# casys-kaist/CoVA

Hardware: AMD Instinct MI355X
Metric: compressed-domain frames/sec (BlobNet+bboxcc) at 1080p b=256 (higher is better)
Workload: dtype f16

## Files before the change

cova_amd/csrc/bboxcc_wave.h:

```cpp
#pragma once
#include <cstdint>

#include "bboxcc_body.h"

#ifdef PHASE_TIMING
__device__ unsigned long long g_ccph[8];
#define CCWG_MARK(i)                                                        \
    do {                                                                    \
        if (tid == 0) {                                                     \
            const unsigned long long now_ = __builtin_amdgcn_s_memrealtime(); \
            atomicAdd(&g_ccph[i], now_ - cc_last_);                         \
            cc_last_ = now_;                                                \
        }                                                                   \
    } while (0)
#else
#define CCWG_MARK(i) do { } while (0)
#endif

namespace ccwave {

struct WvGeom {
    int H, W, BH, BW, NXB;
    int cap;
    int rows_bytes;
// ... 40 lines not shown
__device__ __forceinline__ uint64_t mask_upto(int e) { return e >= 63 ? ~0ull : ((2ull << e) - 1); }

__device__ __forceinline__ int frame_wave(const uint8_t *m, uint8_t *sm, const WvGeom &g, int area_thresh, covahip_box *ob,
                                           int32_t *count_out, int max_boxes, int lane) {
    uint32_t *rows = reinterpret_cast<uint32_t *>(sm);
    uint32_t *lab = reinterpret_cast<uint32_t *>(sm + g.rows_bytes);
    uint32_t *s_area = lab + g.cap, *s_minx = s_area + g.cap, *s_maxx = s_minx + g.cap, *s_miny = s_maxx + g.cap,
             *s_maxy = s_miny + g.cap;

    for (int i = lane; i < g.rows_bytes / 4; i += 64) rows[i] = 0;
    wave_fence();
    const int npieces = g.H * g.NXB;
    constexpr int UN = 8;
    for (int q0 = lane; q0 < npieces; q0 += 64 * UN) {
        uint2 v[UN];
#pragma unroll
        for (int k = 0; k < UN; k++) {
            const int q = q0 + 64 * k;
            v[k] = q < npieces ? *reinterpret_cast<const uint2 *>(m + (size_t)q * 8) : make_uint2(0, 0);
        }
#pragma unroll
        for (int k = 0; k < UN; k++) {
            if ((v[k].x | v[k].y) == 0) continue;
            const int q = q0 + 64 * k;
            const int y = g.mNXB ? (int)__umulhi((uint32_t)q, g.mNXB) : q, xc = q - y * g.NXB;
            const uint32_t tl = nz_bits(v[k].x), th = nz_bits(v[k].y);
            const uint32_t e = (((tl & 0x00800080u) * 0x00800100u) >> 30) | ((((th & 0x00800080u) * 0x00800100u) >> 30) << 2);
            const uint32_t o = (((tl & 0x80008000u) * 0x00008001u) >> 30) | ((((th & 0x80008000u) * 0x00008001u) >> 30) << 2);
            uint32_t *rw = rows + (y + 1) * 4 + (xc >> 3);
            const int sh = 4 * (xc & 7);
            if (e) atomicOr(rw, e << sh);
            if (o) atomicOr(rw + 2, o << sh);
        }
    }

    wave_fence();
    uint64_t a = 0, b = 0, c = 0, d = 0, ue = 0, uo = 0;
    if (lane < g.BH) {
        const uint4 ru = reinterpret_cast<const uint4 *>(rows)[2 * lane];
        const uint4 r0 = reinterpret_cast<const uint4 *>(rows)[2 * lane + 1];
        const uint4 r1 = reinterpret_cast<const uint4 *>(rows)[2 * lane + 2];
        ue = ru.x | ((uint64_t)ru.y << 32); uo = ru.z | ((uint64_t)ru.w << 32);
        a = r0.x | ((uint64_t)r0.y << 32);  b = r0.z | ((uint64_t)r0.w << 32);
        c = r1.x | ((uint64_t)r1.y << 32);  d = r1.z | ((uint64_t)r1.w << 32);
    }
    const uint64_t F = a | b | c | d;
    const uint64_t J = (a | c) & ((b | d) << 1);
    const uint64_t S = F & ~J;
    const int nr = __popcll((unsigned long long)S);
    int incl = nr;
#pragma unroll
    for (int o = 1; o < 64; o <<= 1) {
        const int t = __shfl_up(incl, o, 64);
        if (lane >= o) incl += t;
    }
    const int base = incl - nr;
    const int n = __shfl(incl, 63, 64);
    if (n > g.cap) return n;
    uint64_t S_up = (uint64_t)__shfl_up((unsigned long long)S, 1, 64), J_up = (uint64_t)__shfl_up((unsigned long long)J, 1, 64);
    int base_up = __shfl_up(base, 1, 64);
    if (lane == 0) { S_up = 0; J_up = 0; base_up = 0; }

    for (int i = lane; i < n; i += 64) lab[i] = (uint32_t)i;
    wave_fence();

    {
        const int nhelp = min(64 - g.BH, g.BH);
        const bool helper = lane >= g.BH && lane - g.BH < nhelp;
        const int row = helper ? lane - g.BH : lane;
        const bool split = row < nhelp;
        const uint64_t ha = (uint64_t)__shfl((unsigned long long)a, row, 64), hb = (uint64_t)__shfl((unsigned long long)b, row, 64);
        const uint64_t hc = (uint64_t)__shfl((unsigned long long)c, row, 64), hd = (uint64_t)__shfl((unsigned long long)d, row, 64);
        const uint64_t hue = (uint64_t)__shfl((unsigned long long)ue, row, 64), huo = (uint64_t)__shfl((unsigned long long)uo, row, 64);
        const uint64_t hSu = (uint64_t)__shfl((unsigned long long)S_up, row, 64), hJu = (uint64_t)__shfl((unsigned long long)J_up, row, 64);
        const int hbase = __shfl(base, row, 64), hbase_up = __shfl(base_up, row, 64);
        const uint64_t hJ = (ha | hc) & ((hb | hd) << 1);
        const uint64_t hS = (ha | hb | hc | hd) & ~hJ;
        const uint64_t hcU = (ha | hb) & (hue | huo), hcUL = ha & (huo << 1), hcUR = hb & (hue >> 1);
        uint64_t P = hS;
        P ^= P << 1; P ^= P << 2; P ^= P << 4; P ^= P << 8; P ^= P << 16; P ^= P << 32;
        uint64_t Sr = lane >= g.BH && !helper ? 0 : !split ? hS : helper ? hS & ~P : hS & P;
        while (__any(Sr != 0)) {
            uint64_t Tu = 0;
            int idx = 0;
            if (Sr) {
                const int s = ctz64(Sr);
                Sr &= Sr - 1;
                idx = hbase + __popcll((unsigned long long)(hS & ((1ull << s) - 1)));
                const uint64_t jr = (hJ >> s) >> 1;
                const int e = s + (~jr ? ctz64(~jr) : 0);
                const uint64_t mk = mask_upto(e) & ~((1ull << s) - 1);
                const uint64_t ra = ha & mk, rb = hb & mk, rc = hc & mk, rd = hd & mk;
                s_area[idx] = (uint32_t)(__popcll((unsigned long long)ra) + __popcll((unsigned long long)rb) +
                                         __popcll((unsigned long long)rc) + __popcll((unsigned long long)rd));
                s_minx[idx] = (uint32_t)(2 * s + (((ha | hc) >> s) & 1 ? 0 : 1));
                s_maxx[idx] = (uint32_t)(2 * e + (((hb | hd) >> e) & 1 ? 1 : 0));
                s_miny[idx] = (uint32_t)(2 * row + ((ra | rb) ? 0 : 1));
                s_maxy[idx] = (uint32_t)(2 * row + ((rc | rd) ? 1 : 0));
                Tu = (hcU & mk) | ((hcUL & mk) >> 1) | ((hcUR & mk) << 1);
            }
            while (__any(Tu != 0)) {
                if (Tu) {
                    const int p = ctz64(Tu);
                    const int rank = __popcll((unsigned long long)(hSu << (63 - p))) - 1;
                    const uint64_t jr = (hJu >> p) >> 1;
                    const int e_up = p + (~jr ? ctz64(~jr) : 0);
                    Tu &= ~mask_upto(e_up);
                    ccbody::uf_union(lab, (uint32_t)idx, (uint32_t)(hbase_up + rank));
                }
            }
        }
    }

    wave_fence();
    for (int i = lane; i < n; i += 64) {
        const uint32_t root = ccbody::uf_find(lab, (uint32_t)i);
        if (root != (uint32_t)i) {
            lab[i] = root;
            atomicAdd(&s_area[root], s_area[i]);
            atomicMin(&s_minx[root], s_minx[i]);
            atomicMax(&s_maxx[root], s_maxx[i]);
            atomicMin(&s_miny[root], s_miny[i]);
            atomicMax(&s_maxy[root], s_maxy[i]);
        }
    }
    wave_fence();
    int total = 0;
    for (int i0 = 0; i0 < n; i0 += 64) {
        const int i = i0 + lane;
        const bool keep = i < n && lab[i] == (uint32_t)i && (int)s_area[i] >= area_thresh;
        const uint64_t bal = __ballot(keep);
        if (keep) {
            const int pos = total + __popcll((unsigned long long)(bal & ((1ull << lane) - 1)));
            if (pos < max_boxes) {
                covahip_box bx;
                bx.left = (int32_t)s_minx[i];
                bx.top = (int32_t)s_miny[i];
                bx.width = (int32_t)(s_maxx[i] - s_minx[i] + 1);
                bx.height = (int32_t)(s_maxy[i] - s_miny[i] + 1);
                bx.area_px = (int32_t)s_area[i];
                ob[pos] = bx;
            }
        }
        total += __popcll((unsigned long long)bal);
    }
    if (lane == 0) *count_out = total;
    return n;
}

template <int NTH, bool PLANES = false>
__device__ __forceinline__ void frame_wg(const uint8_t *m, uint8_t *sm, const WvGeom &g, int area_thresh, covahip_box *ob,
                                         int32_t *count_out, int max_boxes, int tid, uint32_t *planes = nullptr) {
    constexpr int NWV = NTH / 64;
    const int lane = tid & 63, wave = tid >> 6;
    uint32_t *rows = PLANES ? planes : reinterpret_cast<uint32_t *>(sm);
    uint32_t *lab = reinterpret_cast<uint32_t *>(sm + g.rows_bytes);
    uint32_t *s_area = lab + g.cap, *s_minx = s_area + g.cap, *s_maxx = s_minx + g.cap, *s_miny = s_maxx + g.cap,
             *s_maxy = s_miny + g.cap;
    __shared__ uint32_t wave_tot[NWV];
#ifdef PHASE_TIMING
    unsigned long long cc_last_ = __builtin_amdgcn_s_memrealtime();
#endif

    if constexpr (!PLANES) {
    for (int i = tid; i < g.rows_bytes / 4; i += NTH) rows[i] = 0;
    __syncthreads();
    const int npieces = g.H * g.NXB;
    for (int q = tid; q < npieces; q += NTH) {
        const uint2 v = *reinterpret_cast<const uint2 *>(__builtin_assume_aligned(m + (size_t)q * 8, 8));
        if ((v.x | v.y) == 0) continue;
        const int y = g.mNXB ? (int)__umulhi((uint32_t)q, g.mNXB) : q, xc = q - y * g.NXB;
        const uint32_t tl = nz_bits(v.x), th = nz_bits(v.y);
        const uint32_t e = (((tl & 0x00800080u) * 0x00800100u) >> 30) | ((((th & 0x00800080u) * 0x00800100u) >> 30) << 2);
        const uint32_t o = (((tl & 0x80008000u) * 0x00008001u) >> 30) | ((((th & 0x80008000u) * 0x00008001u) >> 30) << 2);
        uint32_t *rw = rows + (y + 1) * 4 + (xc >> 3);
        const int sh = 4 * (xc & 7);
        if (e) atomicOr(rw, e << sh);
        if (o) atomicOr(rw + 2, o << sh);
    }
    __syncthreads();
    }
    CCWG_MARK(0);
    uint64_t a = 0, b = 0, c = 0, d = 0, ue = 0, uo = 0;
    if (lane < g.BH) {
        const uint4 ru = reinterpret_cast<const uint4 *>(rows)[2 * lane];
        const uint4 r0 = reinterpret_cast<const uint4 *>(rows)[2 * lane + 1];
        const uint4 r1 = reinterpret_cast<const uint4 *>(rows)[2 * lane + 2];
        ue = ru.x | ((uint64_t)ru.y << 32); uo = ru.z | ((uint64_t)ru.w << 32);
        a = r0.x | ((uint64_t)r0.y << 32);  b = r0.z | ((uint64_t)r0.w << 32);
        c = r1.x | ((uint64_t)r1.y << 32);  d = r1.z | ((uint64_t)r1.w << 32);
    }
    const uint64_t F = a | b | c | d;
    const uint64_t J = (a | c) & ((b | d) << 1);
    const uint64_t S = F & ~J;
    const uint64_t cU = (a | b) & (ue | uo), cUL = a & (uo << 1), cUR = b & (ue >> 1);
    const int nr = __popcll((unsigned long long)S);
    int incl = nr;
#pragma unroll
    for (int o = 1; o < 64; o <<= 1) {
        const int t = __shfl_up(incl, o, 64);
        if (lane >= o) incl += t;
    }
    const int base = incl - nr;
    const int n = __shfl(incl, 63, 64);
    uint64_t S_up = (uint64_t)__shfl_up((unsigned long long)S, 1, 64), J_up = (uint64_t)__shfl_up((unsigned long long)J, 1, 64);
    int base_up = __shfl_up(base, 1, 64);
    if (lane == 0) { S_up = 0; J_up = 0; base_up = 0; }
    for (int i = tid; i < n; i += NTH) lab[i] = (uint32_t)i;
    __syncthreads();
    CCWG_MARK(1);
    for (int k = wave; __any(k < nr); k += NWV) {
        uint64_t Tu = 0;
        const int idx = base + k;
        if (k < nr) {
            const int s = nth_set_bit64(S, k);
            const uint64_t jr = (J >> s) >> 1;
            const int e = s + (~jr ? ctz64(~jr) : 0);
            const uint64_t mk = mask_upto(e) & ~((1ull << s) - 1);
            const uint64_t ra = a & mk, rb = b & mk, rc = c & mk, rd = d & mk;
            s_area[idx] = (uint32_t)(__popcll((unsigned long long)ra) + __popcll((unsigned long long)rb) +
                                     __popcll((unsigned long long)rc) + __popcll((unsigned long long)rd));
            s_minx[idx] = (uint32_t)(2 * s + (((a | c) >> s) & 1 ? 0 : 1));
            s_maxx[idx] = (uint32_t)(2 * e + (((b | d) >> e) & 1 ? 1 : 0));
            s_miny[idx] = (uint32_t)(2 * lane + ((ra | rb) ? 0 : 1));
            s_maxy[idx] = (uint32_t)(2 * lane + ((rc | rd) ? 1 : 0));
            Tu = (cU & mk) | ((cUL & mk) >> 1) | ((cUR & mk) << 1);
        }
        while (__any(Tu != 0)) {
            if (Tu) {
                const int p = ctz64(Tu);
                const int rank = __popcll((unsigned long long)(S_up << (63 - p))) - 1;
                const uint64_t jr = (J_up >> p) >> 1;
                const int e_up = p + (~jr ? ctz64(~jr) : 0);
                Tu &= ~mask_upto(e_up);
                ccbody::uf_union(lab, (uint32_t)idx, (uint32_t)(base_up + rank));
            }
        }
    }
    __syncthreads();
    CCWG_MARK(2);
    for (int i = tid; i < n; i += NTH) {
        const uint32_t root = ccbody::uf_find(lab, (uint32_t)i);
        if (root != (uint32_t)i) {
            lab[i] = root;
            atomicAdd(&s_area[root], s_area[i]);
            atomicMin(&s_minx[root], s_minx[i]);
            atomicMax(&s_maxx[root], s_maxx[i]);
            atomicMin(&s_miny[root], s_miny[i]);
            atomicMax(&s_maxy[root], s_maxy[i]);
        }
    }
    __syncthreads();
    CCWG_MARK(3);
    const int per = (n + NTH - 1) / NTH;
    const int i0 = tid * per;
    uint32_t cnt = 0;
    for (int k = 0; k < per; k++) {
        const int i = i0 + k;
        if (i < n && lab[i] == (uint32_t)i && (int)s_area[i] >= area_thresh) cnt++;
    }
    uint32_t inc2 = cnt;
#pragma unroll
    for (int o = 1; o < 64; o <<= 1) {
        const uint32_t t = __shfl_up(inc2, o, 64);
        if (lane >= o) inc2 += t;
    }
    if (lane == 63) wave_tot[wave] = inc2;
    __syncthreads();
    uint32_t pbase = 0, total = 0;
#pragma unroll
    for (int k = 0; k < NWV; k++) {
        const uint32_t t = wave_tot[k];
        if (k < wave) pbase += t;
        total += t;
    }
    uint32_t pos = pbase + inc2 - cnt;
    for (int k = 0; k < per; k++) {
        const int i = i0 + k;
        if (i < n && lab[i] == (uint32_t)i && (int)s_area[i] >= area_thresh) {
            if ((int)pos < max_boxes) {
                covahip_box bx;
                bx.left = (int32_t)s_minx[i];
                bx.top = (int32_t)s_miny[i];
                bx.width = (int32_t)(s_maxx[i] - s_minx[i] + 1);
                bx.height = (int32_t)(s_maxy[i] - s_miny[i] + 1);
                bx.area_px = (int32_t)s_area[i];
                ob[pos] = bx;
            }
            pos++;
        }
    }
    if (tid == 0) *count_out = (int32_t)total;
    __syncthreads();
    CCWG_MARK(4);
}

}
```

cova_amd/csrc/blobnet_mfma.hip:

```cpp
#include <algorithm>
#include <cmath>
#include <cstdlib>
#include <cstring>
#include <mutex>
#include <type_traits>
#include <utility>
#include <vector>

#include "bboxcc_body.h"
#include "bboxcc_wave.h"
#include "blobnet.h"
#include "covahip_dev.h"

typedef _Float16 half8 __attribute__((ext_vector_type(8)));
typedef _Float16 half4 __attribute__((ext_vector_type(4)));
typedef float f32x16 __attribute__((ext_vector_type(16)));
typedef float f32x4 __attribute__((ext_vector_type(4)));
typedef _Float16 half2v __attribute__((ext_vector_type(2)));

namespace {

constexpr float BN_EPS = 1e-3f;
constexpr int WG = 256;

// ... 1603 lines not shown
    for (int i = tid; i < n_rows + n_cols; i += 512) {
        int piece;
        if (i < n_rows) {
            piece = i < RC ? i : (g.Hi + 1) * RC + (i - RC);
        } else {
            const int j = i - n_rows, y = j / (2 * CPP), k = j % (2 * CPP);
            piece = (y + 1) * RC + (k < CPP ? k : (g.Wi + 1) * CPP + (k - CPP));
        }
        *reinterpret_cast<uint4 *>(tile + piece * 16) = uint4{0, 0, 0, 0};
    }
}
template <int C1, int C2>
__device__ __forceinline__ void dec012_stage(uint8_t *tile, const __half *ss, const DecLvl &g, int wave, int lane, int first) {
    constexpr int C = C1 + C2, CPP = C / 8;
    const int RC = (g.Wi + 2) * CPP, NI = g.Wi * CPP;
    for (int y = (wave + 8 - first) & 7; y < g.Hi; y += 8) {
        const int r = y + 1;
        const __half *rowp = ss + (size_t)y * g.Wi * C2;
        uint8_t *rowl = tile + (r * RC + CPP) * 16;
        for (int q0 = 0; q0 < NI; q0 += 64) {
            const int q = q0 + lane;
            const int px = q / CPP, chp = q % CPP;
            const int cb = (chp ^ swz_eval<CPP>(g.swz, px + 1, r)) * 8;
            if (q < NI && cb >= C1) glds16(rowp + px * C2 + (cb - C1), rowl + q0 * 16);
        }
    }
}

template <int C, int COUT>
struct Dec012W {
    half8 wf[4 * (C / 16)];
    float es[16], eb[16];
};
template <int C, int COUT>
__device__ __forceinline__ void dec012_load(Dec012W<C, COUT> &w, const half8 *wfrag, const float *epi, int wave, int lane) {
    constexpr int MT = 4 * COUT / 32, KSTEPS = 4 * (C / 16);
    const int mtile = wave % MT, kh = lane >> 5;
    asm volatile("" : "+s"(wfrag), "+s"(epi));
#pragma unroll
    for (int ks = 0; ks < KSTEPS; ks++) w.wf[ks] = wfrag[(mtile * KSTEPS + ks) * 64 + lane];
#pragma unroll
    for (int gq = 0; gq < 4; gq++) {
        const int c0 = (mtile * 32 + 8 * gq + 4 * kh) % COUT;
        const float4 sc = *reinterpret_cast<const float4 *>(epi + c0), sh = *reinterpret_cast<const float4 *>(epi + COUT + c0);
        w.es[4 * gq] = sc.x; w.es[4 * gq + 1] = sc.y; w.es[4 * gq + 2] = sc.z; w.es[4 * gq + 3] = sc.w;
        w.eb[4 * gq] = sh.x; w.eb[4 * gq + 1] = sh.y; w.eb[4 * gq + 2] = sh.z; w.eb[4 * gq + 3] = sh.w;
    }
}
template <int C1, int C2, int COUT, int CN>
__device__ __forceinline__ void dec012_block(const uint8_t *lds0, const uint8_t *tile, uint8_t *next_tile, __half *gout, uint8_t *scr_base,
                                             const Dec012W<C1 + C2, COUT> &w, const DecLvl &g, const DecLvl &gn,
                                             int wave, int lane) {
    constexpr int C = C1 + C2, MT = 4 * COUT / 32, PG = 8 / MT;
    constexpr int KC = C / 16, KSTEPS = 4 * KC, CPP = C / 8, PS = C * 2;
    constexpr int AD = C == 128 ? 4 : 8;
    const int mtile = wave % MT, pgroup = wave / MT;
    const int TC = g.Wi + 2, GW = g.Wi + 1, GH = g.Hi + 1;
    const int kh = lane >> 5;
    const half8 (&wf)[KSTEPS] = w.wf;
    const float (&es)[16] = w.es, (&eb)[16] = w.eb;
    const int npos = GH * GW;
    const int ntiles = (npos + 31) / 32;
    for (int tile_i = pgroup; tile_i < ntiles; tile_i += PG) {
        const int q = tile_i * 32 + (lane & 31);
        const int qc = min(q, npos - 1);
        const int u = fdiv(qc, g.mGW), v = qc - u * GW;
        const uint32_t toff = (uint32_t)(uintptr_t)(lds_void *)tile;
        uint32_t pk[4];
#pragma unroll
        for (int tp = 0; tp < 4; tp++) {
            const int yy = u + 1 - (tp >> 1), xx = v + 1 - (tp & 1);
            pk[tp] = (toff + (uint32_t)((yy * TC + xx) * PS)) | (uint32_t)((kh ^ swz_eval<CPP>(g.swz, xx, yy)) << 4);
        }
        auto frag = [&](int ks) -> half8 {
            const int tp = ks / KC, kc = ks % KC;
            typedef const __attribute__((address_space(3))) half8 *lds_half8_ptr;
            return *(lds_half8_ptr)(uintptr_t)(pk[tp] ^ (uint32_t)(kc << 5));
        };
        half8 ring[AD];
#pragma unroll
        for (int ks = 0; ks < AD; ks++) ring[ks] = frag(ks);
        f32x16 acc;
#pragma unroll
        for (int r = 0; r < 16; r++) acc[r] = 0.f;
#pragma unroll
        for (int ks = 0; ks < KSTEPS; ks++) {
            acc = __builtin_amdgcn_mfma_f32_32x32x16_f16(wf[ks], ring[ks % AD], acc, 0, 0, 0);
            if (ks + AD < KSTEPS) ring[ks % AD] = frag(ks + AD);
        }
        __builtin_amdgcn_sched_group_barrier(0x100, AD, 0);
#pragma unroll
        for (int ks = 0; ks < KSTEPS; ks++) {
            __builtin_amdgcn_sched_group_barrier(0x008, 1, 0);
            if (ks + AD < KSTEPS) __builtin_amdgcn_sched_group_barrier(0x100, 1, 0);
        }
        if constexpr (CN > 0) {
            constexpr int CPPN = CN / 8, PSN = CN * 2;
            const int TCN = gn.Wi + 2;
            static_assert(COUT >= 32 && COUT % 32 == 0, "one output pixel per lane and tile");
            const int nb = mtile * 32 + 4 * kh;
            const int phase = nb / COUT, cob = nb % COUT;
            const int Y = 2 * u + (phase >> 1) - g.cy, X = 2 * v + (phase & 1) - g.cx;
            if (q < npos && Y >= 0 && Y < g.Hd && X >= 0 && X < g.Wd) {
                const int yy = Y + 1, xx = X + 1;
                uint8_t *const pix = next_tile + (yy * TCN + xx) * PSN + (cob & 7) * 2;
                const int sw = swz_eval<CPPN>(gn.swz, xx, yy);
#pragma unroll
                for (int gq = 0; gq < 4; gq++) {
                    half4 o;
#pragma unroll
                    for (int j = 0; j < 4; j++)
                        o[j] = (_Float16)fmaxf(acc[4 * gq + j] * es[4 * gq + j] + eb[4 * gq + j], 0.f);
                    *reinterpret_cast<half4 *>(pix + ((((cob >> 3) + gq) ^ sw) * 16)) = o;
                }
            }
        } else {
            uint8_t *const scr = scr_base + wave * 2048;
            const int pos = lane & 31;
#pragma unroll
            for (int gq = 0; gq < 4; gq++) {
                half4 o;
#pragma unroll
                for (int j = 0; j < 4; j++) o[j] = (_Float16)fmaxf(acc[4 * gq + j] * es[4 * gq + j] + eb[4 * gq + j], 0.f);
                *reinterpret_cast<half4 *>(scr + pos * 64 + ((gq ^ ((pos >> 2) & 3)) * 16) + kh * 8) = o;
            }
            __builtin_amdgcn_fence(__ATOMIC_RELEASE, "wavefront");
            __builtin_amdgcn_wave_barrier();
            __builtin_amdgcn_fence(__ATOMIC_ACQUIRE, "wavefront");
#pragma unroll
            for (int j = 0; j < 2; j++) {
                const int c = j * 64 + lane;
                const int rp = c >> 2;
                const int gq = (c & 3) ^ ((rp >> 2) & 3);
                const int rq = tile_i * 32 + rp;
                if (rq < npos) {
                    const int ru = fdiv(rq, g.mGW), rv = rq - ru * GW;
                    const int n0 = mtile * 32 + 8 * gq;
                    const int phase = n0 / COUT, co0 = n0 % COUT;
                    const int Y = 2 * ru + (phase >> 1) - g.cy, X = 2 * rv + (phase & 1) - g.cx;
                    if (Y >= 0 && Y < g.Hd && X >= 0 && X < g.Wd)
                        *reinterpret_cast<uint4 *>(gout + ((size_t)Y * g.Wd + X) * COUT + co0) =
                            *reinterpret_cast<const uint4 *>(scr + c * 16);
                }
            }
            __builtin_amdgcn_fence(__ATOMIC_RELEASE, "wavefront");
            __builtin_amdgcn_wave_barrier();
        }
    }
}

template <bool MS = false>
__global__ __launch_bounds__(512, 2) void dec012_mfma(Dec012Args p) {
    extern __shared__ __attribute__((aligned(256))) uint8_t smem[];
    const int tid = threadIdx.x, lane = tid & 63, wave = tid >> 6;
    uint8_t *const t0 = smem + p.lv[0].tile_off, *const t1 = smem + p.lv[1].tile_off, *const t2 = smem + p.lv[2].tile_off;
    WGSPAN_BEGIN();
#ifdef PHASE_TIMING
    unsigned long long ph_[9] = {0, 0, 0, 0, 0, 0, 0, 0, 0}, last_ = __builtin_amdgcn_s_memrealtime();
#endif
    dec012_zero_border<128>(t0, p.lv[0], tid);
    dec012_zero_border<128>(t1, p.lv[1], tid);
    dec012_zero_border<64>(t2, p.lv[2], tid);
    for (int b = blockIdx.x; b < p.B; b += gridDim.x) {
        [[maybe_unused]] const uint32_t moff = model_off<MS>(p.model_ids, p.mstride, b);
        if (b != (int)blockIdx.x) lds_barrier();
        PHASE_MARK(0);
        {
            Dec012W<128, 64> w0;
            dec012_load(w0, at_model(p.wf[0], moff), at_model(p.epi[0], moff), wave, lane);
            dec012_stage<0, 128>(t0, p.skip[0] + (size_t)b * p.Ts[0] * p.lv[0].Hi * p.lv[0].Wi * 128, p.lv[0], wave, lane, 0);
            dec012_stage<64, 64>(t1, p.skip[1] + (size_t)b * p.Ts[1] * p.lv[1].Hi * p.lv[1].Wi * 64, p.lv[1], wave, lane, p.lv[0].Hi & 7);
            dec012_stage<32, 32>(t2, p.skip[2] + (size_t)b * p.Ts[2] * p.lv[2].Hi * p.lv[2].Wi * 32, p.lv[2], wave, lane,
                                 (p.lv[0].Hi + p.lv[1].Hi) & 7);
            PHASE_MARK(1);
            wait_vmem();
            lds_barrier();
            PHASE_MARK(2);
            dec012_block<0, 128, 64, 128>(smem, t0, t1, nullptr, nullptr, w0, p.lv[0], p.lv[1], wave, lane);
        }
        PHASE_MARK(3);
        {
            Dec012W<128, 32> w1;
            dec012_load(w1, at_model(p.wf[1], moff), at_model(p.epi[1], moff), wave, lane);
            lds_barrier();
#ifdef PHASE_TIMING
            asm volatile("s_waitcnt vmcnt(0)" ::: "memory");
#endif
            PHASE_MARK(4);
            dec012_block<64, 64, 32, 64>(smem, t1, t2, nullptr, nullptr, w1, p.lv[1], p.lv[2], wave, lane);
        }
        PHASE_MARK(5);
        {
            Dec012W<64, 16> w2;
            dec012_load(w2, at_model(p.wf[2], moff), at_model(p.epi[2], moff), wave, lane);
            lds_barrier();
#ifdef PHASE_TIMING
            asm volatile("s_waitcnt vmcnt(0)" ::: "memory");
#endif
            PHASE_MARK(6);
            dec012_block<32, 32, 16, 0>(smem, t2, nullptr, p.out + (size_t)b * p.lv[2].Hd * p.lv[2].Wd * 16, smem + p.scr_off, w2,
                                        p.lv[2], p.lv[2], wave, lane);
        }
        PHASE_MARK(7);
    }
#ifdef PHASE_TIMING
    if (tid == 0)
        for (int i = 0; i < 9; i++) atomicAdd(&g_phase[48 + i], ph_[i]);
#endif
    WGSPAN_END(3);
}

struct Dec3ccArgs {
    DecArgs d;
    ccbody::CcGeom g;
    ccwave::WvGeom wg;
    int use_wv;
    covahip_box *boxes;
    int32_t *counts;
    int area_thresh, max_boxes;
    int tile_bytes;
    int mfull_off, cc_off;
    int part_off;
    DecMs ms;
};

template <bool WV, bool PART, bool MS = false, bool POST = false>
__global__ __launch_bounds__(ccbody::CC_THREADS) void dec3cc_mfma(Dec3ccArgs q, PostArg<POST> qp) {
    constexpr int C1 = 16, C2 = PART ? 0 : 16, C = C1 + C2, NW = ccbody::CC_THREADS / 64;
    constexpr int KC = C / 16, KSTEPS = 4 * KC, CPP = C / 8, PS = C * 2;
    extern __shared__ __attribute__((aligned(16))) uint8_t smem[];
    const DecArgs &p = q.d;
    const int tid = threadIdx.x, lane = tid & 63, wave = tid >> 6;
    const int TC = p.Wi + 2;
    const int GW = p.Wi + 1, GH = p.Hi + 1;
    const int kh = lane >> 5;
    float fbias = p.epi[0];
    uint8_t *const mfull = smem + q.mfull_off;
    WGSPAN_BEGIN();
#ifdef PHASE_TIMING
    unsigned long long ph_[9] = {0, 0, 0, 0, 0, 0, 0, 0, 0}, last_ = __builtin_amdgcn_s_memrealtime();
#endif

    for (int b = blockIdx.x; b < p.B; b += gridDim.x) {
        const StackPost sp = stack_post<POST, MS>(qp, q.ms.model_ids, b);
        half8 wf[KSTEPS];
        if constexpr (MS) {
            const uint32_t moff = model_off<MS>(q.ms.model_ids, q.ms.mstride, b);
            fbias = at_model(p.epi, moff)[0];
#pragma unroll
            for (int ks = 0; ks < KSTEPS; ks++) wf[ks] = at_model(p.wfrag, moff)[ks * 64 + lane];
        } else {
#pragma unroll
            for (int ks = 0; ks < KSTEPS; ks++) wf[ks] = p.wfrag[ks * 64 + lane];
        }
        auto stage = [&](int band, uint8_t *buf) {
            const int u0 = band * GH / p.nbands, u1 = (band + 1) * GH / p.nbands;
            const int RC = TC * CPP;
            const int nchunk = (u1 - u0 + 1) * RC;
            const __half *su = p.up + ((size_t)b) * p.Hi * p.Wi * C1;
            const __half *ss = p.skip + ((size_t)b * p.Ts) * p.Hi * p.Wi * C2;
            for (int s0 = wave * 64; s0 < nchunk; s0 += NW * 64) {
                const int sidx = s0 + lane;
                if (sidx < nchunk) {
                    const int r = fdiv(sidx, p.mRC), within = sidx - r * RC;
                    const int c = within / CPP, chp = within % CPP;
                    const int cb = (chp ^ swz_eval<CPP>(p.swz, c, r)) * 8;
                    const int y = u0 - 1 + r, x = c - 1;
                    const void *src = p.zero;
                    if (y >= 0 && y < p.Hi && x >= 0 && x < p.Wi) {
                        const size_t pix = (size_t)y * p.Wi + x;
                        src = (PART || cb < C1) ? (const void *)(su + pix * C1 + cb) : (const void *)(ss + pix * C2 + (cb - C1));
                    }
                    glds16(src, buf + s0 * 16);
                }
            }
        };
        if (b != (int)blockIdx.x) lds_barrier();
        PHASE_MARK(0);
        if constexpr (PART) {
            const uint8_t *ps = reinterpret_cast<const uint8_t *>(p.part) + (size_t)b * GH * GW * 16;
            const int nch = GH * GW;
            for (int s0 = wave * 64; s0 < nch; s0 += NW * 64)
                if (s0 + lane < nch) glds16(ps + (size_t)(s0 + lane) * 16, smem + q.part_off + s0 * 16);
        }
        stage(0, smem);
        PHASE_MARK(1);
        for (int band = 0; band < p.nbands; band++) {
            uint8_t *const cur = smem + (band & 1) * q.tile_bytes;
            wait_vmem();
            lds_barrier();
            PHASE_MARK(2);
            if (band + 1 < p.nbands) stage(band + 1, smem + ((band + 1) & 1) * q.tile_bytes);
            PHASE_MARK(3);
            const int u0 = band * GH / p.nbands, u1 = (band + 1) * GH / p.nbands;
            const int npos = (u1 - u0) * GW;
            const int ntiles = (npos + 31) / 32;
            for (int tile = wave; tile < ntiles; tile += NW) {
                const int qi = tile * 32 + (lane & 31);
                const int qc = min(qi, npos - 1);
                const int ul = fdiv(qc, p.mGW), v = qc - ul * GW;
                f32x16 acc;
#pragma unroll
                for (int r = 0; r < 16; r++) acc[r] = 0.f;
#pragma unroll
                for (int a = 0; a < 2; a++)
#pragma unroll
                    for (int bb = 0; bb < 2; bb++) {
                        const int yy = ul + 1 - a, xx = v + 1 - bb;
                        const int pbase = (yy * TC + xx) * PS;
                        const int s = swz_eval<CPP>(p.swz, xx, yy);
#pragma unroll
                        for (int kc = 0; kc < KC; kc++) {
                            const half8 av = *reinterpret_cast<const half8 *>(cur + pbase + (((kc * 2 + kh) ^ s) * 16));
                            acc = __builtin_amdgcn_mfma_f32_32x32x16_f16(wf[(a * 2 + bb) * KC + kc], av, acc, 0, 0, 0);
                        }
                    }
                if (qi < npos && kh == 0) {
                    const int u = u0 + ul;
                    f32x4 pl = {0.f, 0.f, 0.f, 0.f};
                    if constexpr (PART) pl = reinterpret_cast<const f32x4 *>(smem + q.part_off)[u * GW + v];
#pragma unroll
                    for (int r = 0; r < 4; r++) {
                        const int Y = 2 * u + (r >> 1) - p.cy, X = 2 * v + (r & 1) - p.cx;
                        if (Y >= 0 && Y < p.Hd && X >= 0 && X < p.Wd) {
                            float l = acc[r] + fbias;
                            if constexpr (PART) l += pl[r];
                            if (p.logits) p.logits[((size_t)b * p.Hd + Y) * p.Wd + X] = l;
                            bool fg = l > sp.thr;
                            if constexpr (POST) fg = fg && sp.keep[Y * p.Wd + X];
                            mfull[Y * p.Wd + X] = fg ? 1 : 0;
                        }
                    }
                }
            }
        }
        PHASE_MARK(4);
        lds_barrier();
        PHASE_MARK(5);
        if (p.mask) {
            uint8_t *dst = p.mask + (size_t)b * p.Hd * p.Wd;
            const int nbytes = p.Hd * p.Wd;
            if ((nbytes & 3) == 0 && (reinterpret_cast<uintptr_t>(p.mask) & 3) == 0) {
                for (int i = tid; i < nbytes / 4; i += NW * 64)
                    reinterpret_cast<uint32_t *>(dst)[i] = reinterpret_cast<const uint32_t *>(mfull)[i];
            } else {
                for (int i = tid; i < nbytes; i += NW * 64) dst[i] = mfull[i];
            }
        }
        PHASE_MARK(6);
        const int area = stack_area<POST, MS>(qp, q.ms.model_ids, b, q.area_thresh);
        if constexpr (WV)
            ccwave::frame_wg<ccbody::CC_THREADS>(mfull, smem + q.cc_off, q.wg, area, q.boxes + (size_t)b * q.max_boxes,
                                                 q.counts + b, q.max_boxes, tid);
        else
            ccbody::bboxcc_frame(mfull, smem + q.cc_off, q.g, area, q.boxes + (size_t)b * q.max_boxes, q.counts + b,
                                 q.max_boxes, tid);
        PHASE_MARK(7);
    }
#ifdef PHASE_TIMING
    if (tid == 0)
        for (int i = 0; i < 9; i++) atomicAdd(&g_phase[64 + i], ph_[i]);
#endif
    WGSPAN_END(4);
}

template <bool MS = false, bool POST = false>
__global__ __launch_bounds__(ccbody::CC_THREADS) void dec3cc_rows_mfma(Dec3ccArgs q, PostArg<POST> qp) {
    constexpr int NW = ccbody::CC_THREADS / 64, PS = 32;
    extern __shared__ __attribute__((aligned(16))) uint8_t smem[];
    const DecArgs &p = q.d;
    const int tid = threadIdx.x, lane = tid & 63, wave = tid >> 6;
    const int TC = p.Wi + 2, GW = p.Wi + 1, GH = p.Hi + 1;
    const int kh = lane >> 5, pos = lane & 31;
    const float fbias0 = p.epi[0];
    uint32_t *const planes = reinterpret_cast<uint32_t *>(smem + q.mfull_off);
    const f32x4 *const part = reinterpret_cast<const f32x4 *>(smem + q.part_off);
    WGSPAN_BEGIN();
#ifdef PHASE_TIMING
    unsigned long long ph_[9] = {0, 0, 0, 0, 0, 0, 0, 0, 0}, last_ = __builtin_amdgcn_s_memrealtime();
#endif
    uint32_t lc[2][2];
#pragma unroll
    for (int h = 0; h < 2; h++)
#pragma unroll
        for (int bb = 0; bb < 2; bb++) {
            const int xx = min(32 * h + pos, GW - 1) + 1 - bb;
            lc[h][bb] = (uint32_t)(xx * PS + ((kh ^ ((xx >> 3) & 1)) << 4));
        }
    const int row_b = TC * PS;
    for (int b = blockIdx.x; b < p.B; b += gridDim.x) {
        const uint32_t moff = model_off<MS>(q.ms.model_ids, q.ms.mstride, b);
        const float fbias = MS ? at_model(p.epi, moff)[0] : fbias0;
        const StackPost sp = stack_post<POST, MS>(qp, q.ms.model_ids, b);
        half8 wf[4];
#pragma unroll
        for (int ks = 0; ks < 4; ks++) wf[ks] = (MS ? at_model(p.wfrag, moff) : p.wfrag)[ks * 64 + lane];
        if (b != (int)blockIdx.x) lds_barrier();
        PHASE_MARK(0);
        {
            const uint8_t *ps = reinterpret_cast<const uint8_t *>(p.part) + (size_t)b * GH * GW * 16;
            const int nch = GH * GW;
            for (int s0 = wave * 64; s0 < nch; s0 += NW * 64)
                if (s0 + lane < nch) glds16(ps + (size_t)(s0 + lane) * 16, smem + q.part_off + s0 * 16);
        }
        {
            const __half *su = p.up + (size_t)b * p.Hi * p.Wi * 16;
            const int NI = 2 * p.Wi;
            for (int y = wave; y < p.Hi; y += NW) {
                const __half *rowp = su + (size_t)y * p.Wi * 16;
                uint8_t *rowl = smem + ((y + 1) * TC + 1) * PS;
                for (int q0 = 0; q0 < NI; q0 += 64) {
                    const int qq = q0 + lane, px = qq >> 1;
                    const int cb = ((qq & 1) ^ (((px + 1) >> 3) & 1)) * 8;
                    if (qq < NI) glds16(rowp + px * 16 + cb, rowl + q0 * 16);
                }
            }
            const int n_rows = 4 * TC, n_cols = 4 * p.Hi;
            for (int i = tid; i < n_rows + n_cols; i += NW * 64) {
                int piece;
                if (i < n_rows) {
                    piece = i < 2 * TC ? i : (p.Hi + 1) * 2 * TC + (i - 2 * TC);
                } else {
                    const int j = i - n_rows, y = j >> 2, k = j & 3;
                    piece = (y + 1) * 2 * TC + (k < 2 ? k : (p.Wi + 1) * 2 + (k - 2));
                }
                *reinterpret_cast<uint4 *>(smem + piece * 16) = uint4{0, 0, 0, 0};
            }
            for (int i = tid; i < q.wg.rows_bytes / 4; i += NW * 64) planes[i] = 0;
        }
        PHASE_MARK(1);
        wait_vmem();
        lds_barrier();
        PHASE_MARK(2);
        for (int t = wave; t < 2 * GH; t += NW) {
            const int u = t >> 1, h = t & 1;
            if (32 * h >= GW) continue;
            const uint32_t rb = (uint32_t)(u * row_b);
            const uint32_t a00 = rb + row_b + (h ? lc[1][0] : lc[0][0]), a01 = rb + row_b + (h ? lc[1][1] : lc[0][1]);
            const uint32_t a10 = rb + (h ? lc[1][0] : lc[0][0]), a11 = rb + (h ? lc[1][1] : lc[0][1]);
            f32x16 acc;
#pragma unroll
            for (int r = 0; r < 16; r++) acc[r] = 0.f;
            acc = __builtin_amdgcn_mfma_f32_32x32x16_f16(wf[0], *reinterpret_cast<const half8 *>(smem + a00), acc, 0, 0, 0);
            acc = __builtin_amdgcn_mfma_f32_32x32x16_f16(wf[1], *reinterpret_cast<const half8 *>(smem + a01), acc, 0, 0, 0);
            acc = __builtin_amdgcn_mfma_f32_32x32x16_f16(wf[2], *reinterpret_cast<const half8 *>(smem + a10), acc, 0, 0, 0);
            acc = __builtin_amdgcn_mfma_f32_32x32x16_f16(wf[3], *reinterpret_cast<const half8 *>(smem + a11), acc, 0, 0, 0);
            const int v = 32 * h + pos;
            const bool live = kh == 0 && v < GW;
            const f32x4 pl = part[u * GW + min(v, GW - 1)];
            float l[4];
#pragma unroll
            for (int r = 0; r < 4; r++) l[r] = (acc[r] + fbias) + pl[r];
            if (p.logits && live) {
#pragma unroll
                for (int r = 0; r < 4; r++) {
                    const int Y = 2 * u + (r >> 1) - p.cy, X = 2 * v + (r & 1) - p.cx;
                    if (Y >= 0 && Y < p.Hd && X >= 0 && X < p.Wd) p.logits[((size_t)b * p.Hd + Y) * p.Wd + X] = l[r];
                }
            }
#pragma unroll
            for (int r = 0; r < 4; r++) {
                const uint64_t bits = (uint64_t)(uint32_t)__ballot(live && l[r] > sp.thr) << (32 * h);
                const int Y = 2 * u + (r >> 1) - p.cy, X0 = (r & 1) - p.cx;
                const int pln = X0 & 1, sh = X0 >> 1;
                const int nb = (p.Wd - pln + 1) >> 1;
                uint64_t w = sh >= 0 ? bits << sh : bits >> (-sh);
                w &= nb >= 64 ? ~0ull : ((1ull << nb) - 1);
                if (Y >= 0 && Y < p.Hd && lane == 0) {
                    uint32_t *rw = planes + (Y + 1) * 4 + 2 * pln;
                    if ((uint32_t)w) atomicOr(rw, (uint32_t)w);
                    if ((uint32_t)(w >> 32)) atomicOr(rw + 1, (uint32_t)(w >> 32));
                }
            }
        }
        PHASE_MARK(4);
        lds_barrier();
        if constexpr (POST) {
            for (int i = tid; i < 4 * p.Hd; i += NW * 64) planes[4 + i] &= sp.planes[i];
            lds_barrier();
        }
        PHASE_MARK(5);
        if (p.mask) {
            uint32_t *dst = reinterpret_cast<uint32_t *>(p.mask + (size_t)b * p.Hd * p.Wd);
            const int wq = p.Wd >> 2, nq = p.Hd * wq;
            for (int i = tid; i < nq; i += NW * 64) {
                const int y = fdiv(i, p.mRC), xq = i - y * wq;
                const int bx = 2 * xq;
                const uint32_t *rw = planes + (y + 1) * 4 + (bx >> 5);
                const uint32_t e2 = (rw[0] >> (bx & 31)) & 3u, o2 = (rw[2] >> (bx & 31)) & 3u;
                dst[i] = (e2 & 1u) | ((o2 & 1u) << 8) | ((e2 >> 1) << 16) | ((o2 >> 1) << 24);
            }
        }
        PHASE_MARK(6);
        ccwave::frame_wg<ccbody::CC_THREADS, true>(nullptr, smem + q.cc_off, q.wg, stack_area<POST, MS>(qp, q.ms.model_ids, b, q.area_thresh), q.boxes + (size_t)b * q.max_boxes,
                                                   q.counts + b, q.max_boxes, tid, planes);
        PHASE_MARK(7);
    }
#ifdef PHASE_TIMING
    if (tid == 0)
        for (int i = 0; i < 9; i++) atomicAdd(&g_phase[64 + i], ph_[i]);
#endif
    WGSPAN_END(4);
}

void enc_epilogue(int cout, bool allpos, const float *bias, const float *gamma, const float *beta, const float *mean,
                  const float *var, std::vector<float> &wscale, float *epi) {
    wscale.assign(cout, 1.f);
    for (int c = 0; c < cout; c++) {
        const float sc = gamma[c] / std::sqrt(var[c] + BN_EPS), sh = beta[c] - mean[c] * sc;
        wscale[c] = sc;
        const float bp = bias[c] * sc;
        epi[cout + c] = bp + sh;
        if (allpos) {
            epi[c] = -bp;
            epi[2 * cout + c] = 0.f;
        } else {
            epi[c] = sc >= 0.f ? -bp : -3.0e38f;
            epi[2 * cout + c] = sc >= 0.f ? 3.0e38f : -bp;
        }
    }
}

void prep_enc0(bool allpos, const float *k, const float *bias, const float *gamma, const float *beta, const float *mean,
               const float *var, const float *w1, const float *w2, _Float16 *wfrag, float *epi) {
    std::vector<float> ws;
    enc_epilogue(16, allpos, bias, gamma, beta, mean, var, ws, epi);
    for (int set = 0; set < 2; set++)
        for (int ks = 0; ks < 2; ks++)
            for (int l = 0; l < 64; l++)
                for (int j = 0; j < 8; j++) {
                    const int n = l & 15, g = l >> 4;
                    const int px = 2 * (g & 1) + (j >> 2), ch = j & 3;
                    const int kx = set == 0 ? px - 1 : px;
                    int ky = -1;
                    if (ks == 0) ky = g >> 1;
                    else if ((g >> 1) == 0) ky = 2;
                    float w = 0.f;
                    if (ky >= 0 && kx >= 0 && kx < 3 && ch < 3) w = k[((ky * 3 + kx) * 3 + ch) * 16 + n] * ws[n] / 6.0f;
                    wfrag[((set * 2 + ks) * 64 + l) * 8 + j] = f2h(w);
                }
    std::memcpy(epi + 48, w1, 16 * sizeof(float));
    std::memcpy(epi + 64, w2, 16 * sizeof(float));
}

void prep_enc(bool allpos, int cin, int cout, const float *k, const float *bias, const float *gamma, const float *beta,
              const float *mean, const float *var, const float *w1, const float *w2, _Float16 *wfrag, float *epi) {
    const int NT = cout / 32, KC = cin / 16, KSTEPS = 9 * KC;
    std::vector<float> ws;
    enc_epilogue(cout, allpos, bias, gamma, beta, mean, var, ws, epi);
    for (int nt = 0; nt < NT; nt++)
        for (int ks = 0; ks < KSTEPS; ks++)
            for (int l = 0; l < 64; l++)
                for (int j = 0; j < 8; j++) {
                    const int tap = ks / KC, kc = ks % KC;
                    const int c = kc * 16 + 8 * (l >> 5) + j, n = nt * 32 + (l & 31);
                    wfrag[(((size_t)nt * KSTEPS + ks) * 64 + l) * 8 + j] = f2h(k[((size_t)tap * cin + c) * cout + n] * ws[n]);
                }
    std::memcpy(epi + 3 * cout, w1, 16 * sizeof(float));
    std::memcpy(epi + 3 * cout + 16, w2, 16 * sizeof(float));
}

void prep_enc1w(bool allpos, const float *k, const float *bias, const float *gamma, const float *beta, const float *mean,
                const float *var, _Float16 *wfrag) {
    static const int pairs[5][2] = {{0, 1}, {3, 4}, {6, 7}, {2, 5}, {8, -1}};
    std::vector<float> ws, epi(3 * 32);
    enc_epilogue(32, allpos, bias, gamma, beta, mean, var, ws, epi.data());
    for (int nt = 0; nt < 2; nt++)
        for (int s = 0; s < 5; s++)
            for (int l = 0; l < 64; l++)
                for (int j = 0; j < 8; j++) {
                    const int kg = l >> 4, tap = pairs[s][kg >> 1], c = 8 * (kg & 1) + j, n = nt * 16 + (l & 15);
                    wfrag[(((size_t)nt * 5 + s) * 64 + l) * 8 + j] = f2h(tap < 0 ? 0.f : k[((size_t)tap * 16 + c) * 32 + n] * ws[n]);
                }
}

void prep_dec(int cin, int cout, const float *k, const float *bias, const float *gamma, const float *beta,
              const float *mean, const float *var, _Float16 *wfrag, float *epi) {
    const int NTT = 4 * cout / 32, KC = cin / 16, KSTEPS = 4 * KC;
    for (int nt = 0; nt < NTT; nt++)
        for (int ks = 0; ks < KSTEPS; ks++)
            for (int l = 0; l < 64; l++)
                for (int j = 0; j < 8; j++) {
                    const int tap = ks / KC, kc = ks % KC, a = tap >> 1, bb = tap & 1;
                    const int c = kc * 16 + 8 * (l >> 5) + j, n = nt * 32 + (l & 31);
                    const int phase = n / cout, co = n % cout, py = phase >> 1, px = phase & 1;
                    const int ky = py + 2 * a, kx = px + 2 * bb;
                    wfrag[(((size_t)nt * KSTEPS + ks) * 64 + l) * 8 + j] =
                        f2h(k[(((size_t)ky * 4 + kx) * cout + co) * cin + c]);
                }
    for (int c = 0; c < cout; c++) {
        const float sc = gamma[c] / std::sqrt(var[c] + BN_EPS);
        epi[c] = sc;
        epi[cout + c] = bias[c] * sc + (beta[c] - mean[c] * sc);
    }
}

float final_fold(int cin, int cout, const float *k, const float *fk, int n, int a, int bb, int c) {
    const int ky = (n >> 1) + 2 * a, kx = (n & 1) + 2 * bb;
    double sacc = 0.0;
    for (int o = 0; o < cout; o++) sacc += (double)fk[o] * k[(((size_t)ky * 4 + kx) * cout + o) * cin + c];
    return (float)sacc;
}
void prep_final(int cin, int cout, const float *k, const float *bias, const float *fk, const float *fb,
                _Float16 *wfrag, float *epi, int c0 = 0, int cwin = 0) {
    if (!cwin) cwin = cin;
    const int KC = cwin / 16, KSTEPS = 4 * KC;
    for (int ks = 0; ks < KSTEPS; ks++)
        for (int l = 0; l < 64; l++)
            for (int j = 0; j < 8; j++) {
                const int tap = ks / KC, kc = ks % KC, a = tap >> 1, bb = tap & 1;
                const int c = c0 + kc * 16 + 8 * (l >> 5) + j, n = l & 31;
                wfrag[((size_t)ks * 64 + l) * 8 + j] = f2h(n < 4 ? final_fold(cin, cout, k, fk, n, a, bb, c) : 0.f);
            }
    if (epi) {
        double bsum = fb[0];
        for (int o = 0; o < cout; o++) bsum += (double)fk[o] * bias[o];
        epi[0] = (float)bsum;
    }
}
void prep_tail(int cin, int cout, const float *k, const float *fk, int c0, _Float16 *wfrag) {
    for (int s = 0; s < 2; s++)
        for (int l = 0; l < 64; l++)
            for (int j = 0; j < 8; j++) {
                const int i = l & 15, kg = l >> 4, c = c0 + 8 * (kg & 1) + j;
                wfrag[((size_t)s * 64 + l) * 8 + j] = f2h(i < 4 ? final_fold(cin, cout, k, fk, i, 1 - s, 1 - (kg >> 1), c) : 0.f);
            }
// ... 689 lines not shown
```

Before: 2.437 million.

## Interleave two MFMA tiles per wave and batch plane atomics in dec3cc

The dec3cc row loop now processes two tiles per wave per iteration. All eight LDS operand loads are issued before two interleaved MFMA accumulator chains, which hides MFMA dependency latency. It also skips half-tiles that are empty when GW fits in 32 columns. The per-row ballot results are spread across lanes 0-7 so up to eight atomicOr calls run in one instruction instead of serially from lane 0. Separately, wave indices are made scalar with readfirstlane in three kernels. The cost is higher register pressure from two live accumulators and more complex addressing.

Measured after the change: 2.424 million. About the same (-0.5%).

```diff
diff --git a/cova_amd/csrc/bboxcc_wave.h b/cova_amd/csrc/bboxcc_wave.h
--- a/cova_amd/csrc/bboxcc_wave.h
+++ b/cova_amd/csrc/bboxcc_wave.h
@@ -216,7 +216,7 @@
 __device__ __forceinline__ void frame_wg(const uint8_t *m, uint8_t *sm, const WvGeom &g, int area_thresh, covahip_box *ob,
                                          int32_t *count_out, int max_boxes, int tid, uint32_t *planes = nullptr) {
     constexpr int NWV = NTH / 64;
-    const int lane = tid & 63, wave = tid >> 6;
+    const int lane = tid & 63, wave = __builtin_amdgcn_readfirstlane(tid >> 6);
     uint32_t *rows = PLANES ? planes : reinterpret_cast<uint32_t *>(sm);
     uint32_t *lab = reinterpret_cast<uint32_t *>(sm + g.rows_bytes);
     uint32_t *s_area = lab + g.cap, *s_minx = s_area + g.cap, *s_maxx = s_minx + g.cap, *s_miny = s_maxx + g.cap,
diff --git a/cova_amd/csrc/blobnet_mfma.hip b/cova_amd/csrc/blobnet_mfma.hip
--- a/cova_amd/csrc/blobnet_mfma.hip
+++ b/cova_amd/csrc/blobnet_mfma.hip
@@ -1779,7 +1779,7 @@
 template <bool MS = false>
 __global__ __launch_bounds__(512, 2) void dec012_mfma(Dec012Args p) {
     extern __shared__ __attribute__((aligned(256))) uint8_t smem[];
-    const int tid = threadIdx.x, lane = tid & 63, wave = tid >> 6;
+    const int tid = threadIdx.x, lane = tid & 63, wave = __builtin_amdgcn_readfirstlane(tid >> 6);
     uint8_t *const t0 = smem + p.lv[0].tile_off, *const t1 = smem + p.lv[1].tile_off, *const t2 = smem + p.lv[2].tile_off;
     WGSPAN_BEGIN();
 #ifdef PHASE_TIMING
@@ -1996,7 +1996,7 @@
     constexpr int NW = ccbody::CC_THREADS / 64, PS = 32;
     extern __shared__ __attribute__((aligned(16))) uint8_t smem[];
     const DecArgs &p = q.d;
-    const int tid = threadIdx.x, lane = tid & 63, wave = tid >> 6;
+    const int tid = threadIdx.x, lane = tid & 63, wave = __builtin_amdgcn_readfirstlane(tid >> 6);
     const int TC = p.Wi + 2, GW = p.Wi + 1, GH = p.Hi + 1;
     const int kh = lane >> 5, pos = lane & 31;
     const float fbias0 = p.epi[0];
@@ -2059,19 +2059,15 @@
         wait_vmem();
         lds_barrier();
         PHASE_MARK(2);
-        for (int t = wave; t < 2 * GH; t += NW) {
-            const int u = t >> 1, h = t & 1;
-            if (32 * h >= GW) continue;
+        const int tpr = GW > 32 ? 2 : 1, ntile = tpr * GH;
+        auto tile_addr = [&](int t, uint32_t (&ad)[4]) {
+            const int u = tpr == 2 ? t >> 1 : t, h = tpr == 2 ? t & 1 : 0;
             const uint32_t rb = (uint32_t)(u * row_b);
-            const uint32_t a00 = rb + row_b + (h ? lc[1][0] : lc[0][0]), a01 = rb + row_b + (h ? lc[1][1] : lc[0][1]);
-            const uint32_t a10 = rb + (h ? lc[1][0] : lc[0][0]), a11 = rb + (h ? lc[1][1] : lc[0][1]);
-            f32x16 acc;
-#pragma unroll
-            for (int r = 0; r < 16; r++) acc[r] = 0.f;
-            acc = __builtin_amdgcn_mfma_f32_32x32x16_f16(wf[0], *reinterpret_cast<const half8 *>(smem + a00), acc, 0, 0, 0);
-            acc = __builtin_amdgcn_mfma_f32_32x32x16_f16(wf[1], *reinterpret_cast<const half8 *>(smem + a01), acc, 0, 0, 0);
-            acc = __builtin_amdgcn_mfma_f32_32x32x16_f16(wf[2], *reinterpret_cast<const half8 *>(smem + a10), acc, 0, 0, 0);
-            acc = __builtin_amdgcn_mfma_f32_32x32x16_f16(wf[3], *reinterpret_cast<const half8 *>(smem + a11), acc, 0, 0, 0);
+            ad[0] = rb + row_b + (h ? lc[1][0] : lc[0][0]); ad[1] = rb + row_b + (h ? lc[1][1] : lc[0][1]);
+            ad[2] = rb + (h ? lc[1][0] : lc[0][0]);         ad[3] = rb + (h ? lc[1][1] : lc[0][1]);
+        };
+        auto tile_finish = [&](int t, const f32x16 &acc) {
+            const int u = tpr == 2 ? t >> 1 : t, h = tpr == 2 ? t & 1 : 0;
             const int v = 32 * h + pos;
             const bool live = kh == 0 && v < GW;
             const f32x4 pl = part[u * GW + min(v, GW - 1)];
@@ -2085,20 +2081,41 @@
                     if (Y >= 0 && Y < p.Hd && X >= 0 && X < p.Wd) p.logits[((size_t)b * p.Hd + Y) * p.Wd + X] = l[r];
                 }
             }
+            uint32_t word = 0;
 #pragma unroll
             for (int r = 0; r < 4; r++) {
                 const uint64_t bits = (uint64_t)(uint32_t)__ballot(live && l[r] > sp.thr) << (32 * h);
-                const int Y = 2 * u + (r >> 1) - p.cy, X0 = (r & 1) - p.cx;
+                const int X0 = (r & 1) - p.cx;
                 const int pln = X0 & 1, sh = X0 >> 1;
                 const int nb = (p.Wd - pln + 1) >> 1;
                 uint64_t w = sh >= 0 ? bits << sh : bits >> (-sh);
                 w &= nb >= 64 ? ~0ull : ((1ull << nb) - 1);
-                if (Y >= 0 && Y < p.Hd && lane == 0) {
-                    uint32_t *rw = planes + (Y + 1) * 4 + 2 * pln;
-                    if ((uint32_t)w) atomicOr(rw, (uint32_t)w);
-                    if ((uint32_t)(w >> 32)) atomicOr(rw + 1, (uint32_t)(w >> 32));
-                }
-            }
+                if ((lane >> 1) == r) word = (lane & 1) ? (uint32_t)(w >> 32) : (uint32_t)w;
+            }
+            const int Y = 2 * u + (lane >> 2) - p.cy;
+            if (lane < 8 && word && Y >= 0 && Y < p.Hd) atomicOr(planes + (Y + 1) * 4 + 2 * ((((lane >> 1) & 1) - p.cx) & 1) + (lane & 1), word);
+        };
+        for (int t = wave; t < ntile; t += 2 * NW) {
+            const bool two = t + NW < ntile;
+            const int t2 = two ? t + NW : t;
+            uint32_t ad0[4], ad1[4];
+            tile_addr(t, ad0);
+            tile_addr(t2, ad1);
+            half8 f0[4], f1[4];
+#pragma unroll
+            for (int k = 0; k < 4; k++) f0[k] = *reinterpret_cast<const half8 *>(smem + ad0[k]);
+#pragma unroll
+            for (int k = 0; k < 4; k++) f1[k] = *reinterpret_cast<const half8 *>(smem + ad1[k]);
+            f32x16 acc0, acc1;
+#pragma unroll
+            for (int r = 0; r < 16; r++) acc0[r] = acc1[r] = 0.f;
+#pragma unroll
+            for (int k = 0; k < 4; k++) {
+                acc0 = __builtin_amdgcn_mfma_f32_32x32x16_f16(wf[k], f0[k], acc0, 0, 0, 0);
+                acc1 = __builtin_amdgcn_mfma_f32_32x32x16_f16(wf[k], f1[k], acc1, 0, 0, 0);
+            }
+            tile_finish(t, acc0);
+            if (two) tile_finish(t2, acc1);
         }
         PHASE_MARK(4);
         lds_barrier();
```
